# MingyuKim87/Safe_Denoiser

Hardware: AMD Instinct MI355X
Metric: images/sec (512x512, 50 steps, SD-v1.4 + repellency) (higher is better)
Workload: dtype bf16; 1 GPU; README-default end to end (safree = svf = lra = true, safree_neg_prompt_config.json:26-28): token ids -> CLIP -> SAFREE projection -> DDPM 50 steps x UNet on 3 guidance branches with per-prompt text switching + safe_denoiser.yaml repellency (kernel_fast, M=515, sigma 3.15, scale .33, margin 1.6, window 780<=t<=1000) -> VAE decode -> uint8 512x512 images; SD-v1.4 UNet / CLIP / VAE with random weigh; guidance_branches=3, text_encoder_precision=bf16x3, prompts_per_batch=64, latent_repeat=3, renoise_draws_rank0=3520, parallelism=prompt-shard x1

## Files before the change

### safe_denoiser_amd/csrc/sdn_ffn.hip

```cpp
#include "sdn_gemm_common.h"

namespace sdn_gemm_detail {

#define SDN_STAMP(IDX) {}
#ifdef SDN_FFN_STAMPS
__device__ unsigned long long* g_ffn_stamps = nullptr;
#define SDN_FTS_DECL unsigned long long fts_prev = 0, fts_sum[8] = {0, 0, 0, 0, 0, 0, 0, 0};
#define SDN_FTS_MARK(I)                                                                         \
  {                                                                                             \
    unsigned long long t_;                                                                      \
    asm volatile("s_memtime %0\n\ts_waitcnt lgkmcnt(0)" : "=s"(t_)::"memory");                  \
    if ((I) >= 0) fts_sum[(I) < 0 ? 0 : (I)] += t_ - fts_prev;                                  \
    fts_prev = t_;                                                                              \
  }
#define SDN_FTS_FLUSH                                                                           \
  if (g_ffn_stamps && lane == 0)                                                                \
    for (int i_ = 0; i_ < 8; ++i_) g_ffn_stamps[((long)blockIdx.x * 8 + wid) * 8 + i_] = fts_sum[i_];
#else
#define SDN_FTS_DECL
#define SDN_FTS_MARK(I)
#define SDN_FTS_FLUSH
#endif

struct FfnArgs {
  const void* x;
  const float* stats;
  const void* w1;
  const float* c1; const float* d1;
  const void* w2;
  const float* b2;
  const void* residual;
  void* out;
  float* col_stats;
  int M;
};

#define SDN_FFN_CONTRACT(SA, SW)                                                                                           \
      {                                                                                                                    \
        typename T::v8 fa[2][4], fw[2][2];                                                                                 \
        _Pragma("unroll") for (int i = 0; i < 4; ++i)                                                                      \
          fa[0][i] = *reinterpret_cast<const typename T::v8*>((SA) + lds_off(i * 16 + fr, fq));                            \
        _Pragma("unroll") for (int j = 0; j < 2; ++j)                                                                      \
          fw[0][j] = *reinterpret_cast<const typename T::v8*>((SW) + lds_off(j * 16 + fr, fq));                            \
        _Pragma("unroll") for (int gi = 0; gi < 6; ++gi) {                                                                 \
          const int ks = gi / 3, g = gi % 3, nj = g == 2 ? 1 : 2;                                                          \
          if (gi + 1 < 6) {                                                                                                \
            const int ks1 = (gi + 1) / 3, g1 = (gi + 1) % 3, nj1 = g1 == 2 ? 1 : 2;                                        \
            _Pragma("unroll") for (int j = 0; j < nj1; ++j)                                                                \
              fw[(gi + 1) & 1][j] = *reinterpret_cast<const typename T::v8*>((SW) + lds_off((2 * g1 + j) * 16 + fr, ks1 * 4 + fq)); \
          }                                                                                                                \
          if (gi == 1) {                                                                                                   \
            _Pragma("unroll") for (int i = 0; i < 4; ++i)                                                                  \
              fa[1][i] = *reinterpret_cast<const typename T::v8*>((SA) + lds_off(i * 16 + fr, 4 + fq));                    \
          }                                                                                                                \
          __builtin_amdgcn_s_setprio(1);                                                                                   \
          _Pragma("unroll") for (int i = 0; i < 4; ++i)                                                                    \
            _Pragma("unroll") for (int j = 0; j < nj; ++j)                                                                 \
              acc[i][2 * g + j] = T::mfma16(fw[gi & 1][j], fa[ks][i], acc[i][2 * g + j]);                                  \
          __builtin_amdgcn_s_setprio(0);                                                                                   \
        }                                                                                                                  \
      }

template <typename T>
__global__ void __launch_bounds__(512, 1)
k_ffn320(const FfnArgs a) {
#if defined(__HIP_DEVICE_COMPILE__)
  constexpr int C = 320, HID = 4 * C, KT1 = C / BK, NCH = HID / 64, KT2 = NCH + KT1;
  constexpr int BM = 128, BN = C, THREADS = 512, NWAVES = 8, NREP = 5;
  constexpr int XIMG = BM * 128;
  constexpr int W2IMG = C * 128;
  constexpr int OFF_W2A = KT1 * XIMG;
  constexpr int OFF_RING = OFF_W2A + W2IMG;
  constexpr int LDS_BYTES = OFF_RING + W2IMG;
  constexpr unsigned OOB = 0x80000000u;
  __shared__ __attribute__((aligned(1024))) unsigned char smem[LDS_BYTES];

  const int tid = threadIdx.x, lane = tid & 63;
  const int wid = __builtin_amdgcn_readfirstlane(tid >> 6);
  SDN_FTS_DECL
  SDN_FTS_MARK(-1)
  const int wm = wid >> 2, wn = wid & 3;
  const int lrow = lane >> 3, lchunk = (lane & 7) ^ lrow;
  const int fr = lane & 15, fq = lane >> 4;
  const int m0 = blockIdx.x * BM, n0 = 0;

  const __amdgpu_buffer_rsrc_t rs_x = make_rsrc(a.x, (unsigned)((long)a.M * C * 2));
  const __amdgpu_buffer_rsrc_t rs_w1 = make_rsrc(a.w1, (unsigned)(2 * HID * C * 2));
  const __amdgpu_buffer_rsrc_t rs_w2 = make_rsrc(a.w2, (unsigned)(C * (HID + C) * 2));

#pragma unroll
  for (int q = 0; q < 10; ++q) {
    const int p = wid * 10 + q;
    const int kt = p >> 4, rg = p & 15;
    const int m = m0 + rg * 8 + lrow;
    const unsigned off = m < a.M ? (unsigned)(((long)m * C + kt * BK + lchunk * 8) * 2) : OOB;
    __builtin_amdgcn_raw_ptr_buffer_load_lds(rs_x, (lds_ptr_t)(smem + p * 1024), 16, off, 0, 0, 0);
  }
  const unsigned w1_lane = (unsigned)(((wid * 2 * 8 + lrow) * C + lchunk * 8) * 2);
  auto issue_w1 = [&](int g) {
    const int jc = g / KT1, kt = g - jc * KT1;
    unsigned char* dst = smem + OFF_RING + (g & 1) * XIMG + wid * 2048;
    const unsigned base = w1_lane + (unsigned)((jc * 128 * C + kt * BK) * 2);
    __builtin_amdgcn_raw_ptr_buffer_load_lds(rs_w1, (lds_ptr_t)dst, 16, base, 0, 0, 0);
    __builtin_amdgcn_raw_ptr_buffer_load_lds(rs_w1, (lds_ptr_t)(dst + 1024), 16, base + (unsigned)(8 * C * 2), 0, 0, 0);
  };
  const unsigned w2_lane = (unsigned)(((wid * 5 * 8 + lrow) * (HID + C) + lchunk * 8) * 2);
  auto issue_w2_slice = [&](int t, int q, int buf_off) {
    __builtin_amdgcn_raw_ptr_buffer_load_lds(rs_w2, (lds_ptr_t)(smem + buf_off + (wid * 5 + q) * 1024), 16,
                                             w2_lane + (unsigned)((q * 8 * (HID + C) + t * BK) * 2), 0, 0, 0);
  };

  issue_w1(0);
  f32x4 acc[4][NREP];
  {
    f32x4 bv[NREP];
#pragma unroll
    for (int j = 0; j < NREP; ++j) bv[j] = *reinterpret_cast<const f32x4*>(a.b2 + wn * 16 * NREP + j * 16 + fq * 4);
#pragma unroll
    for (int i = 0; i < 4; ++i)
#pragma unroll
      for (int j = 0; j < NREP; ++j) acc[i][j] = bv[j];
  }
  float ln_mu[4] = {0.f, 0.f, 0.f, 0.f}, ln_rs[4] = {0.f, 0.f, 0.f, 0.f};
  const bool own_stats = a.stats == nullptr;
  if (!own_stats) {
#pragma unroll
    for (int i = 0; i < 4; ++i) {
      const int m = m0 + wm * 64 + i * 16 + fr;
      const float2 st2 = *reinterpret_cast<const float2*>(a.stats + 2 * (long)(m < a.M ? m : 0));
      ln_mu[i] = st2.x; ln_rs[i] = st2.y;
    }
  }
  float ln_s1[4] = {0.f, 0.f, 0.f, 0.f}, ln_s2[4] = {0.f, 0.f, 0.f, 0.f};
  f32x4 cv[2], dv[2];
  auto load_cd = [&](int jc) {
#pragma unroll
    for (int j = 0; j < 2; ++j) {
      const int n = jc * 128 + wn * 32 + j * 16 + fq * 4;
      cv[j] = *reinterpret_cast<const f32x4*>(a.c1 + n); dv[j] = *reinterpret_cast<const f32x4*>(a.d1 + n);
    }
  };
  asm volatile("s_waitcnt vmcnt(0)" ::: "memory");
  __syncthreads();

  const unsigned char* sa_x = smem + (wm * 64) * 128;
  SDN_FTS_MARK(0)
  for (int jc = 0; jc < NCH; ++jc) {
    f32x4 acc1[4][2];
#pragma unroll
    for (int i = 0; i < 4; ++i) { acc1[i][0] = (f32x4){0.f, 0.f, 0.f, 0.f}; acc1[i][1] = (f32x4){0.f, 0.f, 0.f, 0.f}; }
#pragma unroll
    for (int kt = 0; kt < KT1; ++kt) {
      const int g = jc * KT1 + kt;
      if (kt == 0) load_cd(jc);
      if (g + 1 < NCH * KT1) issue_w1(g + 1);
      issue_w2_slice(jc, kt, OFF_W2A);
      const unsigned char* sa = sa_x + kt * XIMG;
      const unsigned char* sw = smem + OFF_RING + (g & 1) * XIMG + (wn * 32) * 128;
#pragma unroll
      for (int ks = 0; ks < 2; ++ks) {
        typename T::v8 fa[4], fw[2];
#pragma unroll
        for (int i = 0; i < 4; ++i) fa[i] = *reinterpret_cast<const typename T::v8*>(sa + lds_off(i * 16 + fr, ks * 4 + fq));
#pragma unroll
        for (int j = 0; j < 2; ++j) fw[j] = *reinterpret_cast<const typename T::v8*>(sw + lds_off(j * 16 + fr, ks * 4 + fq));
        if (own_stats && jc == 0) {
#pragma unroll
          for (int i = 0; i < 4; ++i) { ln_s1[i] = T::dot_ones(fa[i], ln_s1[i]); ln_s2[i] = T::dot_self(fa[i], ln_s2[i]); }
        }
        __builtin_amdgcn_s_setprio(1);
#pragma unroll
        for (int i = 0; i < 4; ++i)
#pragma unroll
          for (int j = 0; j < 2; ++j) acc1[i][j] = T::mfma16(fw[j], fa[i], acc1[i][j]);
        __builtin_amdgcn_s_setprio(0);
      }
      SDN_FTS_MARK(1)
      if (kt + 1 < KT1) asm volatile("s_waitcnt vmcnt(1)" ::: "memory");
      else asm volatile("s_waitcnt vmcnt(0)" ::: "memory");
      asm volatile("s_waitcnt lgkmcnt(0)" ::: "memory");
      SDN_FTS_MARK(2)
      __builtin_amdgcn_s_barrier();
      SDN_FTS_MARK(3)
    }
    if (own_stats && jc == 0) {
      const float invk = 1.0f / (float)C;
#pragma unroll
      for (int i = 0; i < 4; ++i) {
        float a1 = ln_s1[i], a2 = ln_s2[i];
        a1 += __shfl_xor(a1, 16, 64); a2 += __shfl_xor(a2, 16, 64);
        a1 += __shfl_xor(a1, 32, 64); a2 += __shfl_xor(a2, 32, 64);
        const float mu = a1 * invk;
        const float var = fmaxf(a2 * invk - mu * mu, 0.f);
        ln_mu[i] = mu; ln_rs[i] = __builtin_amdgcn_rsqf(var + 1e-5f);
      }
    }
    unsigned char* sh = smem + OFF_RING + ((jc * KT1 + KT1 - 1) & 1) * XIMG;
#pragma unroll
    for (int i = 0; i < 4; ++i) {
      const int row = wm * 64 + i * 16 + fr;
      const float mu = ln_mu[i], rs = ln_rs[i];
      const f32x4 hv = (acc1[i][0] - mu * cv[0]) * rs + dv[0], gv = (acc1[i][1] - mu * cv[1]) * rs + dv[1];
      uint2 pk;
      pk.x = T::pack2(hv[0] * gelu_erf(gv[0]), hv[1] * gelu_erf(gv[1]));
      pk.y = T::pack2(hv[2] * gelu_erf(gv[2]), hv[3] * gelu_erf(gv[3]));
      *reinterpret_cast<uint2*>(sh + lds_off(row, wn * 2 + (fq >> 1)) + (fq & 1) * 8) = pk;
    }
    SDN_FTS_MARK(4)
    __syncthreads();
    SDN_FTS_MARK(5)
    {
      const unsigned char* sa = sh + (wm * 64) * 128;
      const unsigned char* sw = smem + OFF_W2A + (wn * 16 * NREP) * 128;
      SDN_FFN_CONTRACT(sa, sw)
    }
    SDN_FTS_MARK(6)
    __syncthreads();
    SDN_FTS_MARK(5)
  }

  const __amdgpu_buffer_rsrc_t rs_res = make_rsrc(a.residual, (unsigned)((long)a.M * C * 2));
  auto issue_residual = [&](int img) {
#pragma unroll
    for (int q = 0; q < 2; ++q) {
      const int piece = img * 16 + wid * 2 + q;
      const int e = piece * 64 + lane;
      const int r = e / (BN / 8), c = e - r * (BN / 8);
      const int m = m0 + r;
      const unsigned off = m < a.M ? (unsigned)(((long)m * C + c * 8) * 2) : OOB;
      __builtin_amdgcn_raw_ptr_buffer_load_lds(rs_res, (lds_ptr_t)(smem + piece * 1024), 16, off, 0, 0, 0);
    }
  };
#pragma unroll
  for (int q = 0; q < 5; ++q) issue_w2_slice(NCH, q, OFF_W2A);
#pragma unroll
  for (int q = 0; q < 5; ++q) issue_w2_slice(NCH + 1, q, OFF_RING);
#pragma unroll
  for (int kt = 0; kt < KT1; ++kt) {
    const int boff = (kt & 1) ? OFF_RING : OFF_W2A;
    if (kt == 0) asm volatile("s_waitcnt vmcnt(5)" ::: "memory");
    else if (kt == 1) asm volatile("s_waitcnt vmcnt(7)" ::: "memory");
    else if (kt == 2 || kt == 3) asm volatile("s_waitcnt vmcnt(9)" ::: "memory");
    else asm volatile("s_waitcnt vmcnt(4)" ::: "memory");
    __builtin_amdgcn_s_barrier();
    {
      const unsigned char* sa = sa_x + kt * XIMG;
      const unsigned char* sw = smem + boff + (wn * 16 * NREP) * 128;
      SDN_FFN_CONTRACT(sa, sw)
    }
    asm volatile("s_waitcnt lgkmcnt(0)" ::: "memory");
    __builtin_amdgcn_s_barrier();
    if (kt + 2 < KT1) {
#pragma unroll
      for (int q = 0; q < 5; ++q) issue_w2_slice(NCH + kt + 2, q, boff);
    }
    issue_residual(kt);
  }
  asm volatile("s_waitcnt vmcnt(0)" ::: "memory");
  __syncthreads();

  GemmArgs g{};
  g.M = a.M; g.N = C; g.K = HID + C; g.ldc = C; g.n_valid = C; g.act = 0; g.out_kind = 0;
  g.residual = (const __bf16*)a.residual; g.out = a.out; g.col_stats = a.col_stats; g.res_lds = 1;
  g.res_bytes = (unsigned)((long)a.M * C * 2); g.rows_per_batch = 0; g.residual_bcast = 0;
  constexpr int LNF = 0, WGM = 2, NSTAGE = 2, STAGE = LDS_BYTES / 2;
  constexpr int CW_PAD = (BN + 8) * 2;
  const bool staged = true;
  const int out_cols = BN;
  const bool res_lds = true;
  const int CW = BN * 2;
  const bool lean = true, lean_gelu = false, lean_gate = false;
  constexpr int PASSES = 1, WM_PER_PASS = WGM / PASSES, ROWS_PER_PASS = 64 * WM_PER_PASS;
  static_assert(BM * CW_PAD <= NSTAGE * STAGE - 8 * BN * 8, "staged tile and the column-sum scratch must fit the LDS");
#define SDN_EPI_RES_PRELOADED
#define SDN_PASS 0
#include "sdn_gemm_epilogue.inc"
#undef SDN_PASS
#undef SDN_EPI_RES_PRELOADED
  SDN_FTS_MARK(7)
  SDN_FTS_FLUSH
  (void)NWAVES; (void)WGM; (void)lean_gelu; (void)lean_gate; (void)staged; (void)CW_PAD; (void)KT2;
#endif
}

}
using namespace sdn_gemm_detail;

#ifdef SDN_FFN_STAMPS
extern "C" int sdn_debug_set_ffn_stamps(void* p) { return (int)hipMemcpyToSymbol(HIP_SYMBOL(sdn_gemm_detail::g_ffn_stamps), &p, sizeof(p)); }
#endif
extern "C" int sdn_ffn_geglu_fused(int32_t dtype, int64_t M, int32_t C, const void* x, const float* row_stats, const void* w1_folded, const float* c1,
                        const float* d1, const void* w_cat, const float* b_cat, const void* residual, void* out, float* col_stats,
                        void* stream) {
  auto al16 = [](const void* p) { return (reinterpret_cast<uintptr_t>(p) & 15) == 0; };
  if (dtype < 0 || dtype > 1 || C != 320 || M < 0 || !x || !w1_folded || !c1 || !d1 || !w_cat || !b_cat || !residual || !out)
    return SDN_E_INVALID;
  if (!al16(x) || !al16(w1_folded) || !al16(c1) || !al16(d1) || !al16(w_cat) || !al16(b_cat) || !al16(residual) || !al16(out) ||
      (reinterpret_cast<uintptr_t>(row_stats) & 7) || (reinterpret_cast<uintptr_t>(col_stats) & 7))
    return SDN_E_INVALID;
  if (M * C * 2 >= (1L << 31)) return SDN_E_INVALID;
  if (M == 0) return SDN_OK;
  FfnArgs a{x, row_stats, w1_folded, c1, d1, w_cat, b_cat, residual, out, col_stats, (int)M};
  const unsigned grid = (unsigned)((M + 127) / 128);
  record_gemm_launch(4, dtype, 10, 2, 2, row_stats ? 2 : 1, (int)grid, 1, 1, 0);
  if (dtype == 1) hipLaunchKernelGGL((k_ffn320<SdnF16>), dim3(grid), dim3(512), 0, (hipStream_t)stream, a);
  else hipLaunchKernelGGL((k_ffn320<SdnBF16>), dim3(grid), dim3(512), 0, (hipStream_t)stream, a);
  return sdn_launch_status();
}
```

Before: 8.164 images/sec.

## Triple-buffer W1 tiles in fused FFN320 kernel with split W2 slice placement

Changes the W1 weight ring in the fused LayerNorm-GEGLU-FFN kernel for C=320 from two stages to three, so W1 loads are issued two k-tiles ahead. To fit in LDS, the W2 chunk buffer is cut into 64-row slices. The fifth slice goes into a free ring stage, and the contraction reads W2 through per-fragment base pointers. The waitcnt schedule and the ring rotation per chunk change to match, adding a full vmcnt(0) drain before the GEGLU sync. This is meant to hide global-to-LDS latency for W1 in the first GEMM, at the cost of more complex buffer indexing and some added out-of-bounds dummy loads.

```diff
diff --git a/safe_denoiser_amd/csrc/sdn_ffn.hip b/safe_denoiser_amd/csrc/sdn_ffn.hip
--- a/safe_denoiser_amd/csrc/sdn_ffn.hip
+++ b/safe_denoiser_amd/csrc/sdn_ffn.hip
@@ -35,19 +35,19 @@
   int M;
 };
 
-#define SDN_FFN_CONTRACT(SA, SW)                                                                                           \
+#define SDN_FFN_CONTRACT(SA, SWB)                                                                                          \
       {                                                                                                                    \
         typename T::v8 fa[2][4], fw[2][2];                                                                                 \
         _Pragma("unroll") for (int i = 0; i < 4; ++i)                                                                      \
           fa[0][i] = *reinterpret_cast<const typename T::v8*>((SA) + lds_off(i * 16 + fr, fq));                            \
         _Pragma("unroll") for (int j = 0; j < 2; ++j)                                                                      \
-          fw[0][j] = *reinterpret_cast<const typename T::v8*>((SW) + lds_off(j * 16 + fr, fq));                            \
+          fw[0][j] = *reinterpret_cast<const typename T::v8*>((SWB)[j] + lds_off(fr, fq));                                 \
         _Pragma("unroll") for (int gi = 0; gi < 6; ++gi) {                                                                 \
           const int ks = gi / 3, g = gi % 3, nj = g == 2 ? 1 : 2;                                                          \
           if (gi + 1 < 6) {                                                                                                \
             const int ks1 = (gi + 1) / 3, g1 = (gi + 1) % 3, nj1 = g1 == 2 ? 1 : 2;                                        \
             _Pragma("unroll") for (int j = 0; j < nj1; ++j)                                                                \
-              fw[(gi + 1) & 1][j] = *reinterpret_cast<const typename T::v8*>((SW) + lds_off((2 * g1 + j) * 16 + fr, ks1 * 4 + fq)); \
+              fw[(gi + 1) & 1][j] = *reinterpret_cast<const typename T::v8*>((SWB)[2 * g1 + j] + lds_off(fr, ks1 * 4 + fq));   \
           }                                                                                                                \
           if (gi == 1) {                                                                                                   \
             _Pragma("unroll") for (int i = 0; i < 4; ++i)                                                                  \
@@ -70,8 +70,11 @@
   constexpr int XIMG = BM * 128;
   constexpr int W2IMG = C * 128;
   constexpr int OFF_W2A = KT1 * XIMG;
-  constexpr int OFF_RING = OFF_W2A + W2IMG;
-  constexpr int LDS_BYTES = OFF_RING + W2IMG;
+  constexpr int W2SLICE = 64 * 128;
+  constexpr int OFF_RING = OFF_W2A + 4 * W2SLICE;
+  constexpr int OFF_TAILB = OFF_W2A + W2IMG;
+  constexpr int LDS_BYTES = OFF_RING + 3 * XIMG;
+  static_assert(OFF_TAILB + W2IMG == LDS_BYTES, "the trailing k-tiles double-buffer 40 KB weight tiles behind X");
   constexpr unsigned OOB = 0x80000000u;
   __shared__ __attribute__((aligned(1024))) unsigned char smem[LDS_BYTES];
 
@@ -97,20 +100,21 @@
     __builtin_amdgcn_raw_ptr_buffer_load_lds(rs_x, (lds_ptr_t)(smem + p * 1024), 16, off, 0, 0, 0);
   }
   const unsigned w1_lane = (unsigned)(((wid * 2 * 8 + lrow) * C + lchunk * 8) * 2);
-  auto issue_w1 = [&](int g) {
+  auto issue_w1 = [&](int g, int stage) {
     const int jc = g / KT1, kt = g - jc * KT1;
-    unsigned char* dst = smem + OFF_RING + (g & 1) * XIMG + wid * 2048;
+    unsigned char* dst = smem + OFF_RING + stage * XIMG + wid * 2048;
+    const bool live = g < NCH * KT1;
     const unsigned base = w1_lane + (unsigned)((jc * 128 * C + kt * BK) * 2);
-    __builtin_amdgcn_raw_ptr_buffer_load_lds(rs_w1, (lds_ptr_t)dst, 16, base, 0, 0, 0);
-    __builtin_amdgcn_raw_ptr_buffer_load_lds(rs_w1, (lds_ptr_t)(dst + 1024), 16, base + (unsigned)(8 * C * 2), 0, 0, 0);
+    __builtin_amdgcn_raw_ptr_buffer_load_lds(rs_w1, (lds_ptr_t)dst, 16, live ? base : OOB, 0, 0, 0);
+    __builtin_amdgcn_raw_ptr_buffer_load_lds(rs_w1, (lds_ptr_t)(dst + 1024), 16, live ? base + (unsigned)(8 * C * 2) : OOB, 0, 0, 0);
   };
-  const unsigned w2_lane = (unsigned)(((wid * 5 * 8 + lrow) * (HID + C) + lchunk * 8) * 2);
-  auto issue_w2_slice = [&](int t, int q, int buf_off) {
-    __builtin_amdgcn_raw_ptr_buffer_load_lds(rs_w2, (lds_ptr_t)(smem + buf_off + (wid * 5 + q) * 1024), 16,
-                                             w2_lane + (unsigned)((q * 8 * (HID + C) + t * BK) * 2), 0, 0, 0);
+  const unsigned w2_lane = (unsigned)(((wid * 8 + lrow) * (HID + C) + lchunk * 8) * 2);
+  auto issue_w2_slice = [&](int t, int q, unsigned char* dst) {
+    __builtin_amdgcn_raw_ptr_buffer_load_lds(rs_w2, (lds_ptr_t)(dst + wid * 1024), 16,
+                                             w2_lane + (unsigned)((q * 64 * (HID + C) + t * BK) * 2), 0, 0, 0);
   };
 
-  issue_w1(0);
+  issue_w1(0, 0);
   f32x4 acc[4][NREP];
   {
     f32x4 bv[NREP];
@@ -145,18 +149,23 @@
 
   const unsigned char* sa_x = smem + (wm * 64) * 128;
   SDN_FTS_MARK(0)
+  int s0 = 0;
   for (int jc = 0; jc < NCH; ++jc) {
+    auto stage_of = [&](int kt) { const int s = s0 + kt % 3; return s >= 3 ? s - 3 : s; };
     f32x4 acc1[4][2];
 #pragma unroll
     for (int i = 0; i < 4; ++i) { acc1[i][0] = (f32x4){0.f, 0.f, 0.f, 0.f}; acc1[i][1] = (f32x4){0.f, 0.f, 0.f, 0.f}; }
 #pragma unroll
     for (int kt = 0; kt < KT1; ++kt) {
       const int g = jc * KT1 + kt;
-      if (kt == 0) load_cd(jc);
-      if (g + 1 < NCH * KT1) issue_w1(g + 1);
-      issue_w2_slice(jc, kt, OFF_W2A);
+      if (kt == 0) {
+        load_cd(jc);
+        issue_w1(g + 1, stage_of(1));
+      }
+      if (kt + 1 < KT1) issue_w1(g + 2, stage_of(kt + 2));
+      issue_w2_slice(jc, kt, kt + 1 < KT1 ? smem + OFF_W2A + kt * W2SLICE : smem + OFF_RING + stage_of(3) * XIMG);
       const unsigned char* sa = sa_x + kt * XIMG;
-      const unsigned char* sw = smem + OFF_RING + (g & 1) * XIMG + (wn * 32) * 128;
+      const unsigned char* sw = smem + OFF_RING + stage_of(kt) * XIMG + (wn * 32) * 128;
 #pragma unroll
       for (int ks = 0; ks < 2; ++ks) {
         typename T::v8 fa[4], fw[2];
@@ -176,8 +185,8 @@
         __builtin_amdgcn_s_setprio(0);
       }
       SDN_FTS_MARK(1)
-      if (kt + 1 < KT1) asm volatile("s_waitcnt vmcnt(1)" ::: "memory");
-      else asm volatile("s_waitcnt vmcnt(0)" ::: "memory");
+      if (kt == 0) asm volatile("s_waitcnt vmcnt(3)" ::: "memory");
+      else if (kt + 1 < KT1) asm volatile("s_waitcnt vmcnt(4)" ::: "memory");
       asm volatile("s_waitcnt lgkmcnt(0)" ::: "memory");
       SDN_FTS_MARK(2)
       __builtin_amdgcn_s_barrier();
@@ -195,7 +204,7 @@
         ln_mu[i] = mu; ln_rs[i] = __builtin_amdgcn_rsqf(var + 1e-5f);
       }
     }
-    unsigned char* sh = smem + OFF_RING + ((jc * KT1 + KT1 - 1) & 1) * XIMG;
+    unsigned char* sh = smem + OFF_RING + stage_of(KT1 - 1) * XIMG;
 #pragma unroll
     for (int i = 0; i < 4; ++i) {
       const int row = wm * 64 + i * 16 + fr;
@@ -207,16 +216,24 @@
       *reinterpret_cast<uint2*>(sh + lds_off(row, wn * 2 + (fq >> 1)) + (fq & 1) * 8) = pk;
     }
     SDN_FTS_MARK(4)
+    asm volatile("s_waitcnt vmcnt(0)" ::: "memory");
     __syncthreads();
     SDN_FTS_MARK(5)
     {
       const unsigned char* sa = sh + (wm * 64) * 128;
-      const unsigned char* sw = smem + OFF_W2A + (wn * 16 * NREP) * 128;
-      SDN_FFN_CONTRACT(sa, sw)
+      const unsigned char* sw4 = smem + OFF_RING + stage_of(3) * XIMG;
+      const unsigned char* swb[NREP];
+#pragma unroll
+      for (int j = 0; j < NREP; ++j) {
+        const int r0 = (wn * NREP + j) * 16;
+        swb[j] = r0 < 4 * 64 ? smem + OFF_W2A + r0 * 128 : sw4 + (r0 - 4 * 64) * 128;
+      }
+      SDN_FFN_CONTRACT(sa, swb)
     }
     SDN_FTS_MARK(6)
     __syncthreads();
     SDN_FTS_MARK(5)
+    s0 = s0 == 0 ? 2 : s0 - 1;
   }
 
   const __amdgpu_buffer_rsrc_t rs_res = make_rsrc(a.residual, (unsigned)((long)a.M * C * 2));
@@ -232,12 +249,12 @@
     }
   };
 #pragma unroll
-  for (int q = 0; q < 5; ++q) issue_w2_slice(NCH, q, OFF_W2A);
-#pragma unroll
-  for (int q = 0; q < 5; ++q) issue_w2_slice(NCH + 1, q, OFF_RING);
+  for (int q = 0; q < 5; ++q) issue_w2_slice(NCH, q, smem + OFF_W2A + q * W2SLICE);
+#pragma unroll
+  for (int q = 0; q < 5; ++q) issue_w2_slice(NCH + 1, q, smem + OFF_TAILB + q * W2SLICE);
 #pragma unroll
   for (int kt = 0; kt < KT1; ++kt) {
-    const int boff = (kt & 1) ? OFF_RING : OFF_W2A;
+    const int boff = (kt & 1) ? OFF_TAILB : OFF_W2A;
     if (kt == 0) asm volatile("s_waitcnt vmcnt(5)" ::: "memory");
     else if (kt == 1) asm volatile("s_waitcnt vmcnt(7)" ::: "memory");
     else if (kt == 2 || kt == 3) asm volatile("s_waitcnt vmcnt(9)" ::: "memory");
@@ -245,14 +262,16 @@
     __builtin_amdgcn_s_barrier();
     {
       const unsigned char* sa = sa_x + kt * XIMG;
-      const unsigned char* sw = smem + boff + (wn * 16 * NREP) * 128;
-      SDN_FFN_CONTRACT(sa, sw)
+      const unsigned char* swb[NREP];
+#pragma unroll
+      for (int j = 0; j < NREP; ++j) swb[j] = smem + boff + ((wn * NREP + j) * 16) * 128;
+      SDN_FFN_CONTRACT(sa, swb)
     }
     asm volatile("s_waitcnt lgkmcnt(0)" ::: "memory");
     __builtin_amdgcn_s_barrier();
     if (kt + 2 < KT1) {
 #pragma unroll
-      for (int q = 0; q < 5; ++q) issue_w2_slice(NCH + kt + 2, q, boff);
+      for (int q = 0; q < 5; ++q) issue_w2_slice(NCH + kt + 2, q, smem + boff + q * W2SLICE);
     }
     issue_residual(kt);
   }
```

Result: no change. 8.169 images/sec (median of 2 runs) (+0.1%).
